# ronghanghu/vit_10b_fsdp_example

Measured on NVIDIA H100. Metric: vit10b images/sec (device-timed, max over ranks), higher is better.
Workload: dtype bf16

## Files before the change

### vit_10b_fsdp_example_b200/csrc/bindings.cpp

```cpp
#include <ATen/cuda/CUDAContext.h>
#include <c10/cuda/CUDAGuard.h>
#include <torch/extension.h>

#include <cmath>
#include <optional>
#include <vector>

#include "attention_sm90.h"
#include "comm.h"
#include "elementwise.h"
#include "gemm_sm90.h"
#include "layer_scale.h"
#include "patch_drop.h"
#include "prefix_tokens.h"

namespace {

using torch::Tensor;
using OptT = std::optional<Tensor>;

inline const __nv_bfloat16* bf16_ptr(const Tensor& t) {
    TORCH_CHECK(t.is_cuda(), "expected a CUDA tensor");
    TORCH_CHECK(t.scalar_type() == at::kBFloat16, "expected a bf16 tensor");
    return reinterpret_cast<const __nv_bfloat16*>(t.data_ptr());
}
inline __nv_bfloat16* bf16_mut(Tensor& t) { return const_cast<__nv_bfloat16*>(bf16_ptr(t)); }
inline float* f32_ptr(const Tensor& t) {
    TORCH_CHECK(t.is_cuda() && t.scalar_type() == at::kFloat, "expected a CUDA fp32 tensor");
    return reinterpret_cast<float*>(t.data_ptr());
}
inline cudaStream_t cur_stream() { return at::cuda::getCurrentCUDAStream().stream(); }

void gemm(Tensor a, int64_t lda, int64_t major_a, Tensor b, int64_t ldb, int64_t major_b, Tensor d, int64_t ldd,
          int64_t M, int64_t N, int64_t K, OptT bias, OptT residual, int64_t ld_res, int64_t res_row_mod, OptT aux_in,
          int64_t ld_aux, OptT aux_out, int64_t ld_aux_out, OptT colsum, int64_t colsum_bi_stride, int64_t act,
          std::vector<int64_t> batch, int64_t block_n, int64_t cluster, int64_t max_ctas, std::vector<int64_t> ag,
          OptT row_scale, int64_t rows_per_scale) {
    c10::cuda::CUDAGuard guard(a.device());
    b200::GemmOperand A, B, D, X;
    A.ptr = bf16_ptr(a), A.ld = lda;
    B.ptr = bf16_ptr(b), B.ld = ldb;
    D.ptr = bf16_ptr(d), D.ld = ldd;
    if (!batch.empty()) {
        TORCH_CHECK(batch.size() == 8, "batch spec must have 8 entries");
        A.nb_inner = B.nb_inner = D.nb_inner = batch[0];
        A.nb_outer = B.nb_outer = D.nb_outer = batch[1];
        A.stride_b_inner = batch[2], A.stride_b_outer = batch[3];
        B.stride_b_inner = batch[4], B.stride_b_outer = batch[5];
        D.stride_b_inner = batch[6], D.stride_b_outer = batch[7];
    }
    b200::GemmEpilogue e;
    if (bias.has_value()) e.bias = bf16_ptr(*bias);
    if (residual.has_value()) e.residual = bf16_ptr(*residual), e.ld_res = ld_res, e.res_row_mod = (int)res_row_mod;
    if (aux_in.has_value()) e.aux_in = bf16_ptr(*aux_in), e.ld_aux = ld_aux;
    if (colsum.has_value()) e.colsum = f32_ptr(*colsum), e.colsum_bi_stride = colsum_bi_stride;
    e.act = static_cast<int>(act);
    if (row_scale.has_value()) {
        TORCH_CHECK(row_scale->is_contiguous() && row_scale->numel() * rows_per_scale >= M,
                    "gemm: row_scale must be contiguous with one entry per rows_per_scale rows");
        e.row_scale = f32_ptr(*row_scale), e.rows_per_scale = (int)rows_per_scale;
    }
    if (aux_out.has_value()) {
        X = D;
        X.ptr = bf16_ptr(*aux_out), X.ld = ld_aux_out;
        e.has_aux_out = 1;
    }
    b200::GemmAgFuse fuse;
    if (!ag.empty()) {
        TORCH_CHECK(ag.size() >= 6 && (int64_t)ag.size() == 6 + ag[0] && ag[0] <= 16, "bad AG-fusion spec");
        fuse.world = (int)ag[0], fuse.rank = (int)ag[1], fuse.rows_per_slab = (int)ag[2], fuse.slab_bytes = ag[3];
        fuse.dst = reinterpret_cast<void*>(ag[4]);
        fuse.flags = reinterpret_cast<uint32_t*>(ag[5]);
        for (int64_t r = 0; r < ag[0]; ++r) fuse.peer_src[r] = static_cast<uint64_t>(ag[6 + r]);
    }
    b200::gemm_bf16(A, (int)major_a, B, (int)major_b, D, aux_out.has_value() ? &X : nullptr, (int)M, (int)N, (int)K, e,
                    (int)block_n, (int)cluster, (int)max_ctas, cur_stream(), ag.empty() ? nullptr : &fuse);
}

void layernorm_fwd(Tensor x, Tensor gamma, Tensor beta, Tensor y, Tensor mean, Tensor rstd, double eps) {
    c10::cuda::CUDAGuard guard(x.device());
    const int D = (int)x.size(-1);
    const int rows = (int)(x.numel() / D);
    b200::layernorm_fwd(bf16_ptr(x), bf16_ptr(gamma), bf16_ptr(beta), bf16_mut(y), f32_ptr(mean), f32_ptr(rstd), rows,
                        D, (float)eps, cur_stream());
}

void layernorm_bwd(Tensor dy, Tensor x, Tensor gamma, Tensor mean, Tensor rstd, OptT dres, Tensor dx, Tensor dgamma,
                   Tensor dbeta, OptT dxsum) {
    c10::cuda::CUDAGuard guard(x.device());
    const int D = (int)x.size(-1);
    const int rows = (int)(x.numel() / D);
    b200::layernorm_bwd(bf16_ptr(dy), bf16_ptr(x), bf16_ptr(gamma), f32_ptr(mean), f32_ptr(rstd),
                        dres.has_value() ? bf16_ptr(*dres) : nullptr, bf16_mut(dx), f32_ptr(dgamma), f32_ptr(dbeta),
                        dxsum.has_value() ? f32_ptr(*dxsum) : nullptr, rows, D, cur_stream());
}

void softmax_fwd(Tensor s, int64_t rows, int64_t n, int64_t ld, double scale) {
    c10::cuda::CUDAGuard guard(s.device());
    b200::softmax_fwd(bf16_mut(s), rows, (int)n, ld, (float)scale, cur_stream());
}
void softmax_bwd(Tensor dp, Tensor p, int64_t rows, int64_t n, int64_t ld, double scale) {
    c10::cuda::CUDAGuard guard(p.device());
    b200::softmax_bwd(bf16_mut(dp), bf16_ptr(p), rows, (int)n, ld, (float)scale, cur_stream());
}

bool attention_supported(int64_t N, int64_t hd) { return b200::attention_supported((int)N, (int)hd); }

void attention_fwd(Tensor qkv, Tensor out, OptT lse, OptT probs, int64_t B, int64_t N, int64_t H, int64_t hd,
                   double drop_p, int64_t drop_key) {
// ... 488 lines not shown
```

### vit_10b_fsdp_example_b200/csrc/gemm_sm90.cu

```cuda
#include <cuda.h>
#include <cuda_runtime.h>
#include <cuda_bf16.h>
#include <cstdint>
#include <cstdio>
#include <cstdlib>
#include <cstring>
#include <mutex>
#include <stdexcept>
#include <string>
#include <algorithm>
#include <unordered_map>

#include "gemm_sm90.h"
#include "ptx.cuh"
#include "wgmma.cuh"

namespace b200 {

namespace {

constexpr int kBlockM = 128;
constexpr int kBlockK = 64;
constexpr int kMmaK = 16;
constexpr int kConsumerWgs = 2;
// ... 30 lines not shown
    uint32_t v;
    asm volatile("ld.acquire.gpu.global.u32 %0, [%1];" : "=r"(v) : "l"(ptr) : "memory");
    return v;
}
__device__ __forceinline__ void fence_proxy_async_all() { asm volatile("fence.proxy.async;" ::: "memory"); }

__device__ __forceinline__ float rcp_approx(float x) {
    float r;
    asm("rcp.approx.ftz.f32 %0, %1;" : "=f"(r) : "f"(x));
    return r;
}
__device__ __forceinline__ float erf_as(float z, float& e) {
    const float az = fabsf(z);
    const float t = rcp_approx(fmaf(0.3275911f, az, 1.0f));
    e = __expf(-az * az);
    float poly = fmaf(1.061405429f, t, -1.453152027f);
    poly = fmaf(poly, t, 1.421413741f);
    poly = fmaf(poly, t, -0.284496736f);
    poly = fmaf(poly, t, 0.254829592f);
    const float y = 1.0f - poly * t * e;
    return copysignf(y, z);
}
__device__ __forceinline__ float gelu_erf(float x) {
    float e;
    return 0.5f * x * (1.0f + erf_as(x * 0.70710678118654752f, e));
}
__device__ __forceinline__ float dgelu_erf(float x) {
    float e;
    const float cdf = 0.5f * (1.0f + erf_as(x * 0.70710678118654752f, e));
    return fmaf(x * 0.3989422804014327f, e, cdf);
}
__device__ __forceinline__ float sigmoid_approx(float x) { return rcp_approx(1.0f + __expf(-x)); }

template <int kMajorA, int kMajorB, int BLOCK_N, int kStages, int kClusterM, bool kRowScale, int kGlu>
__device__ __forceinline__ void gemm_bf16_sm90_body(const CUtensorMap& tmap_a, const CUtensorMap& tmap_b,
                                                    const CUtensorMap& tmap_d, const CUtensorMap& tmap_aux,
                                                    const KernelParams& p) {
    constexpr int kABytes = kBlockM * kBlockK * 2;
    constexpr int kBBytes = BLOCK_N * kBlockK * 2;
    constexpr int kStageBytes = kABytes + kBBytes;
    constexpr int kTileN = kGlu == kActSwiglu ? BLOCK_N / 2 : BLOCK_N;
    static_assert(BLOCK_N % 64 == 0 && BLOCK_N <= 256, "epilogue works in 64-column chunks; wgmma N <= 256");
    static_assert(kABytes % 1024 == 0 && kBBytes % 1024 == 0, "swizzle-128B needs 1024 B aligned stages");
    static_assert(kClusterM == 1 || (kClusterM == 2 && BLOCK_N % 128 == 0), "B splits into two 64-row multiples");
    static_assert(kGlu != kActSwiglu || (kMajorA == 0 && kMajorB == 0 && BLOCK_N % 128 == 0 && !kRowScale),
                  "SwiGLU forward: K-major operands, gate / value halves of 64-row multiples");
    static_assert(kGlu != kActDSwiglu || (kMajorA == 0 && kMajorB == 1 && !kRowScale), "dSwiGLU: the fc2 dgrad (NN)");

    extern __shared__ __align__(1024) uint8_t smem[];
    uint8_t* smem_cd = smem;
    uint8_t* smem_a = smem + kCdBufs * kCdBufBytes;
    uint8_t* smem_b = smem_a + kStages * kABytes;
    uint64_t* full_bar = reinterpret_cast<uint64_t*>(smem_b + kStages * kBBytes);
    uint64_t* empty_bar = full_bar + kStages;

    const uint32_t warp_idx = threadIdx.x / 32;
    const uint32_t lane = lane_id();
    const uint32_t wg = warp_idx / 4;
    if (threadIdx.x == 0 && (smem_u32(smem) & 1023u) != 0) __trap();

    if (warp_idx == 0 && elect_one()) {
        prefetch_tmap(&tmap_a);
        prefetch_tmap(&tmap_b);
        prefetch_tmap(&tmap_d);
        if (p.epi.has_aux_out) prefetch_tmap(&tmap_aux);
        for (int i = 0; i < kStages; ++i) {
            mbar_init(&full_bar[i], 1);
            mbar_init(&empty_bar[i], kConsumerWgs * 4 * kClusterM);
        }
        fence_mbar_init();
    }
    if constexpr (kClusterM > 1)
        cluster_sync();
    else
        __syncthreads();

    auto cta_rank = [] { return kClusterM > 1 ? static_cast<int>(cluster_ctarank()) : 0; };
    const int units_per_batch = p.m_units * p.n_tiles;
    const int total_units = units_per_batch * p.batch;
    const int num_kb = (p.K + kBlockK - 1) / kBlockK;
    const int kGroupN = p.group_n;

    auto decode_tile = [&](int t, int& b, int& mt, int& nt) {
        b = t / units_per_batch;
        const int r = t - b * units_per_batch;
        const int per_group = p.m_units * kGroupN;
        const int g = r / per_group;
        const int first_n = g * kGroupN;
        const int gsz = min(kGroupN, p.n_tiles - first_n);
        const int in_g = r - g * per_group;
        mt = (in_g / gsz) * kClusterM + cta_rank();
        nt = first_n + in_g % gsz;
        nt += p.n_rot;
        if (nt >= p.n_tiles) nt -= p.n_tiles;
    };
    const int ag_chunks_per_slab =
        p.ag.world > 1 ? static_cast<int>((p.ag.slab_bytes + kAgChunkBytes - 1) / kAgChunkBytes) : 0;

    if (wg == 0) {
        reg_dealloc<56>();
        if (warp_idx == 0) {
            if (elect_one()) {
                uint32_t stage = 0, phase = 0;
                for (int t = blockIdx.x / kClusterM; t < total_units; t += gridDim.x / kClusterM) {
                    int b, mt, nt;
                    decode_tile(t, b, mt, nt);
                    const int bi = b % p.nb_inner, bo = b / p.nb_inner;
                    const int m_idx = mt * kBlockM;
                    const int n_idx = nt * kTileN;
                    if (p.ag.world > 1) {
                        const int last_row = min(n_idx + BLOCK_N, p.N) - 1;
                        if (last_row >= n_idx) {
                            const int s_lo = min(n_idx / p.ag.rows_per_slab, p.ag.world - 1);
                            const int s_hi = min(last_row / p.ag.rows_per_slab, p.ag.world - 1);
                            for (int sl = s_lo; sl <= s_hi; ++sl) {
                                uint32_t spins = 0;
                                while (ld_acquire_gpu(p.ag.flags + sl) < static_cast<uint32_t>(ag_chunks_per_slab)) {
                                    if (++spins > (1u << 26)) __trap();
                                }
                            }
                            fence_proxy_async_all();
                        }
                    }
                    for (int kb = 0; kb < num_kb; ++kb) {
                        mbar_wait_silent(&empty_bar[stage], phase ^ 1);
                        const int k_idx = kb * kBlockK;
                        uint8_t* sa = smem_a + stage * kABytes;
                        uint8_t* sb = smem_b + stage * kBBytes;
                        mbar_arrive_expect_tx(&full_bar[stage], kStageBytes);
                        if constexpr (kMajorA == 0) {
                            tma_load_4d(&tmap_a, &full_bar[stage], sa, k_idx, m_idx, bi, bo);
                        } else {
#pragma unroll
                            for (int i = 0; i < kBlockM / 64; ++i)
                                tma_load_4d(&tmap_a, &full_bar[stage], sa + i * (64 * kBlockK * 2), m_idx + i * 64,
                                                 k_idx, bi, bo);
                        }
                        if constexpr (kGlu == kActSwiglu) {
                            constexpr int kHalfN = BLOCK_N / 2;
                            if constexpr (kClusterM == 1) {
                                tma_load_4d(&tmap_b, &full_bar[stage], sb, k_idx, n_idx, bi, bo);
                                tma_load_4d(&tmap_b, &full_bar[stage], sb + kHalfN * (kBlockK * 2), k_idx, p.N + n_idx,
                                            bi, bo);
                            } else {
                                const int r = cta_rank();
                                tma_load_4d_multicast(&tmap_b, &full_bar[stage], sb + r * kHalfN * (kBlockK * 2), k_idx,
                                                      n_idx + r * p.N, bi, bo, 0b11);
                            }
                        } else if constexpr (kClusterM == 1) {
                            if constexpr (kMajorB == 0) {
                                tma_load_4d(&tmap_b, &full_bar[stage], sb, k_idx, n_idx, bi, bo);
                            } else {
#pragma unroll
                                for (int i = 0; i < BLOCK_N / 64; ++i)
                                    tma_load_4d(&tmap_b, &full_bar[stage], sb + i * (64 * kBlockK * 2), n_idx + i * 64,
                                                k_idx, bi, bo);
                            }
                        } else {
                            constexpr int kHalfN = BLOCK_N / 2;
                            const int h = cta_rank() * kHalfN;
                            if constexpr (kMajorB == 0) {
                                tma_load_4d_multicast(&tmap_b, &full_bar[stage], sb + h * (kBlockK * 2), k_idx,
                                                      n_idx + h, bi, bo, 0b11);
                            } else {
#pragma unroll
                                for (int i = 0; i < kHalfN / 64; ++i)
                                    tma_load_4d_multicast(&tmap_b, &full_bar[stage],
// ... 32 lines not shown
                    }
                    for (; i < nvec; i += 32) *reinterpret_cast<uint4*>(dst + static_cast<int64_t>(i) * 16) = ld_peer_v4(src + static_cast<int64_t>(i) * 16);
                    __threadfence();
                    __syncwarp();
                    if (lane == 0) red_release_gpu_add(p.ag.flags + sl, 1);
                }
            }
        }
    } else {
        reg_alloc<224>();
        const uint32_t cw = wg - 1;
        const uint32_t etid = threadIdx.x & 127;
        const uint32_t wrow = (warp_idx & 3) * 16 + lane / 4;
        const uint32_t cpair = (lane & 3) * 2;
        const uint32_t bar_id = 1 + cw;
        uint8_t* const grp_buf = smem_cd + cw * 2 * kCdBufBytes;
        const GemmEpilogue& e = p.epi;
        const bool ext_is_aux = e.act == kActDGelu;
        constexpr uint32_t kLbo = kBlockK * 128;
        constexpr uint32_t kKStepA = kMajorA == 0 ? (kMmaK * 2) : (kMmaK * 128);
        constexpr uint32_t kKStepB = kMajorB == 0 ? (kMmaK * 2) : (kMmaK * 128);
        constexpr uint32_t kSlabA = 64 * kBlockK * 2;
        uint32_t stage = 0, phase = 0;
        uint32_t flip = 0;
        float d[BLOCK_N / 2];
        auto release = [&](uint32_t s) {
            if constexpr (kClusterM == 1) {
                mbar_arrive(&empty_bar[s]);
            } else {
#pragma unroll
                for (int c = 0; c < kClusterM; ++c) mbar_arrive_cluster(&empty_bar[s], c);
            }
        };

        for (int t = blockIdx.x / kClusterM; t < total_units; t += gridDim.x / kClusterM) {
            int b, mt, nt;
            decode_tile(t, b, mt, nt);
            const int bi = b % p.nb_inner, bo = b / p.nb_inner;
            const int m0 = mt * kBlockM + cw * 64;
            const int n0 = nt * kTileN;

            uint32_t prev_stage = 0;
            for (int kb = 0; kb < num_kb; ++kb) {
                mbar_wait_silent(&full_bar[stage], phase);
                const uint32_t a_addr = smem_u32(smem_a + stage * kABytes) + cw * kSlabA;
                const uint32_t b_addr = smem_u32(smem_b + stage * kBBytes);
                wgmma_fence();
#pragma unroll
                for (int k = 0; k < kBlockK / kMmaK; ++k) {
                    const uint64_t da = make_wgmma_desc(a_addr + k * kKStepA, kLbo, 1024, 1);
                    const uint64_t db = make_wgmma_desc(b_addr + k * kKStepB, kLbo, 1024, 1);
                    WgmmaSS<BLOCK_N, kMajorA, kMajorB>::mma(d, da, db, (kb > 0 || k > 0) ? 1u : 0u);
                }
                wgmma_commit();
                if (kb > 0) {
                    wgmma_wait<1>();
                    if (lane == 0) release(prev_stage);
                }
                prev_stage = stage;
                stage = (stage + 1 == kStages) ? 0 : stage + 1;
                phase ^= (stage == 0);
            }
            wgmma_wait<0>();
            if (lane == 0) release(prev_stage);

            const int row0 = m0 + static_cast<int>(wrow), row1 = row0 + 8;
            const bool row0_ok = row0 < p.M, row1_ok = row1 < p.M;
            if constexpr (kGlu == kActSwiglu) {
                constexpr int kHalfChunks = BLOCK_N / 128;
                auto gate_value = [&](int c, int j, float (&a)[4], float (&v)[4]) {
#pragma unroll
                    for (int q = 0; q < 4; ++q) a[q] = d[(c * 8 + j) * 4 + q], v[q] = d[((c + kHalfChunks) * 8 + j) * 4 + q];
                };
#pragma unroll
                for (int c = 0; c < kHalfChunks; ++c) {
                    const int ncol0 = n0 + c * 64;
                    if (ncol0 >= p.N) continue;
                    if (e.bias != nullptr) {
#pragma unroll
                        for (int j = 0; j < 8; ++j) {
                            const int col = ncol0 + j * 8 + static_cast<int>(cpair);
                            if (col < p.N) {
                                const uint32_t bg = __ldg(reinterpret_cast<const uint32_t*>(e.bias + col));
                                const uint32_t bv = __ldg(reinterpret_cast<const uint32_t*>(e.bias + p.N + col));
                                float* dg = d + (c * 8 + j) * 4;
                                float* dv = d + ((c + kHalfChunks) * 8 + j) * 4;
                                dg[0] += bf16_lo(bg), dg[1] += bf16_hi(bg), dg[2] += bf16_lo(bg), dg[3] += bf16_hi(bg);
                                dv[0] += bf16_lo(bv), dv[1] += bf16_hi(bv), dv[2] += bf16_lo(bv), dv[3] += bf16_hi(bv);
                            }
                        }
                    }
                    if (e.has_aux_out) {
                        if (etid == 0) tma_store_wait_read<0>();
                        named_bar_sync(bar_id, kEpiThreads);
#pragma unroll
                        for (int j = 0; j < 8; ++j) {
                            float a[4], v[4];
// ... 193 lines not shown
                            s += __bfloat162float(*reinterpret_cast<const __nv_bfloat16*>(ptr));
                        }
                        if (ncol0 + ccol < p.N)
                            atomicAdd(e.colsum + static_cast<int64_t>(bi) * e.colsum_bi_stride + ncol0 + ccol, s);
                    }
                    ++flip;
                }
            }
        }
        if (etid == 0) tma_store_wait<0>();
    }
    if constexpr (kClusterM > 1) {
        __syncwarp();
        cluster_sync();
    }
}

template <int kMajorA, int kMajorB, int BLOCK_N, int kStages, int kClusterM, bool kRowScale>
__global__ void __launch_bounds__(kNumThreads, 1)
    gemm_bf16_sm90_kernel(const __grid_constant__ CUtensorMap tmap_a, const __grid_constant__ CUtensorMap tmap_b,
                          const __grid_constant__ CUtensorMap tmap_d, const __grid_constant__ CUtensorMap tmap_aux,
                          const KernelParams p) {
    gemm_bf16_sm90_body<kMajorA, kMajorB, BLOCK_N, kStages, kClusterM, kRowScale, 0>(tmap_a, tmap_b, tmap_d, tmap_aux, p);
}

template <int kMajorB, int BLOCK_N, int kStages, int kClusterM, int kGlu>
__global__ void __launch_bounds__(kNumThreads, 1)
    gemm_glu_sm90_kernel(const __grid_constant__ CUtensorMap tmap_a, const __grid_constant__ CUtensorMap tmap_b,
                         const __grid_constant__ CUtensorMap tmap_d, const __grid_constant__ CUtensorMap tmap_aux,
                         const KernelParams p) {
    gemm_bf16_sm90_body<0, kMajorB, BLOCK_N, kStages, kClusterM, false, kGlu>(tmap_a, tmap_b, tmap_d, tmap_aux, p);
}

using EncodeFn = CUresult (*)(CUtensorMap*, CUtensorMapDataType, cuuint32_t, void*, const cuuint64_t*,
                              const cuuint64_t*, const cuuint32_t*, const cuuint32_t*, CUtensorMapInterleave,
                              CUtensorMapSwizzle, CUtensorMapL2promotion, CUtensorMapFloatOOBfill);

EncodeFn get_encode_fn() {
    static EncodeFn fn = nullptr;
    static std::once_flag once;
    std::call_once(once, [] {
        void* sym = nullptr;
        cudaDriverEntryPointQueryResult qres;
        cudaError_t err = cudaGetDriverEntryPoint("cuTensorMapEncodeTiled", &sym, cudaEnableDefault, &qres);
        if (err != cudaSuccess || qres != cudaDriverEntryPointSuccess || sym == nullptr)
            throw std::runtime_error("cuTensorMapEncodeTiled not available from the driver");
        fn = reinterpret_cast<EncodeFn>(sym);
    });
    return fn;
}

struct TmapKey {
    uint64_t ptr;
    int64_t d[4];
    int64_t s[3];
    int32_t box[2];
    bool operator==(const TmapKey& o) const { return std::memcmp(this, &o, sizeof(TmapKey)) == 0; }
};
struct TmapKeyHash {
    size_t operator()(const TmapKey& k) const {
        const uint64_t* w = reinterpret_cast<const uint64_t*>(&k);
        size_t h = 1469598103934665603ull;
        for (size_t i = 0; i < sizeof(TmapKey) / 8; ++i) h = (h ^ w[i]) * 1099511628211ull;
        return h;
    }
};
// ... 29 lines not shown
                                   box, estr, CU_TENSOR_MAP_INTERLEAVE_NONE,
                                   swizzle_bytes == 128 ? CU_TENSOR_MAP_SWIZZLE_128B
                                   : swizzle_bytes == 64 ? CU_TENSOR_MAP_SWIZZLE_64B
                                                         : CU_TENSOR_MAP_SWIZZLE_32B,
                                   CU_TENSOR_MAP_L2_PROMOTION_L2_256B, CU_TENSOR_MAP_FLOAT_OOB_FILL_NONE);
    if (res != CUDA_SUCCESS) {
        char msg[256];
        snprintf(msg, sizeof(msg),
                 "cuTensorMapEncodeTiled failed (%d): dims=(%lld,%lld,%lld,%lld) ld=%lld box=(%d,%d)", (int)res,
                 (long long)inner, (long long)outer, (long long)op.nb_inner, (long long)op.nb_outer, (long long)op.ld,
                 box_inner, box_outer);
        throw std::runtime_error(msg);
    }
    std::lock_guard<std::mutex> lock(mu);
    if (cache.size() > 4096) cache.clear();
    cache.emplace(key, tm);
    return tm;
}

int num_sms() {
    static int n = 0;
    if (n == 0) {
        int dev = 0;
        cudaGetDevice(&dev);
        cudaDeviceGetAttribute(&n, cudaDevAttrMultiProcessorCount, dev);
    }
    return n;
}

void check(cudaError_t err, const char* what) {
    if (err != cudaSuccess) throw std::runtime_error(std::string(what) + ": " + cudaGetErrorString(err));
}

template <int kMajorA, int kMajorB, int BLOCK_N, int kStages, int kClusterM, bool kRowScale, int kGlu>
constexpr auto kernel_for() {
    if constexpr (kGlu == 0)
        return gemm_bf16_sm90_kernel<kMajorA, kMajorB, BLOCK_N, kStages, kClusterM, kRowScale>;
    else
        return gemm_glu_sm90_kernel<kMajorB, BLOCK_N, kStages, kClusterM, kGlu>;
}

template <int kMajorA, int kMajorB, int BLOCK_N, int kStages, int kClusterM, bool kRowScale = false, int kGlu = 0>
void launch(const GemmOperand& A, const GemmOperand& B, const GemmOperand& D, const GemmOperand* aux, int M, int N,
            int K, const GemmEpilogue& epi, int max_ctas, cudaStream_t stream, const GemmAgFuse* ag) {
    constexpr int kSmem = kCdBufs * kCdBufBytes + kStages * (kBlockM + BLOCK_N) * kBlockK * 2 + 2 * kStages * 8;
    static_assert(kSmem <= 232448, "shared memory budget exceeded (227 KB per block on sm_90)");
    constexpr int kTileN = kGlu == kActSwiglu ? BLOCK_N / 2 : BLOCK_N;
    auto kern = kernel_for<kMajorA, kMajorB, BLOCK_N, kStages, kClusterM, kRowScale, kGlu>();
    static bool attr_set = false;
    if (!attr_set) {
        check(cudaFuncSetAttribute(kern, cudaFuncAttributeMaxDynamicSharedMemorySize, kSmem), "cudaFuncSetAttribute");
        attr_set = true;
    }
    cudaLaunchConfig_t cfg = {};
    cudaLaunchAttribute cluster_attr;
    cluster_attr.id = cudaLaunchAttributeClusterDimension;
    cluster_attr.val.clusterDim.x = kClusterM, cluster_attr.val.clusterDim.y = 1, cluster_attr.val.clusterDim.z = 1;
    cfg.blockDim = dim3(kNumThreads);
    cfg.dynamicSmemBytes = kSmem;
    cfg.stream = stream;
    cfg.attrs = &cluster_attr;
    cfg.numAttrs = kClusterM > 1 ? 1 : 0;
    static int resident_units = 0;
    if (resident_units == 0) {
        if constexpr (kClusterM == 1) {
            resident_units = num_sms();
        } else {
            cfg.gridDim = dim3(num_sms() / kClusterM * kClusterM);
            check(cudaOccupancyMaxActiveClusters(&resident_units, kern, &cfg), "cudaOccupancyMaxActiveClusters");
            if (resident_units < 1) throw std::runtime_error("gemm: no 2-CTA cluster of this kernel fits an SM pair");
        }
    }
    CUtensorMap ta = kMajorA == 0 ? make_tmap(A, K, M, kBlockK, kBlockM) : make_tmap(A, M, K, 64, kBlockK);
    CUtensorMap tb = kGlu == kActSwiglu ? make_tmap(B, K, 2 * static_cast<int64_t>(N), kBlockK, BLOCK_N / 2)
                     : kMajorB == 0     ? make_tmap(B, K, N, kBlockK, BLOCK_N / kClusterM)
                                        : make_tmap(B, N, K, 64, kBlockK);
    CUtensorMap td = make_tmap(D, N, M, 64, 64);
    CUtensorMap tx = td;
    if (epi.has_aux_out && aux != nullptr) {
        GemmOperand x = *aux;
        if (kGlu == kActSwiglu) x.nb_inner = 2, x.stride_b_inner = N;
        tx = make_tmap(x, N, M, 64, 64);
    }

    KernelParams p;
    p.M = M, p.N = N, p.K = K;
    p.batch = static_cast<int>(D.nb_inner * D.nb_outer);
    p.nb_inner = static_cast<int>(D.nb_inner);
    p.m_tiles = (M + kBlockM - 1) / kBlockM;
    p.m_units = (p.m_tiles + kClusterM - 1) / kClusterM;
    p.n_tiles = (N + kTileN - 1) / kTileN;
    p.epi = epi;
    p.n_rot = 0;
    p.group_n = 2048 / BLOCK_N;
    if (ag != nullptr && ag->world > 1) {
        if (kMajorB != 0 || p.batch != 1) throw std::runtime_error("gemm: AG fusion needs a K-major, un-batched B");
        if (static_cast<int64_t>(ag->rows_per_slab) * K * 2 != ag->slab_bytes || ag->slab_bytes % 16 != 0)
            throw std::runtime_error("gemm: AG fusion needs whole rows per slab");
        p.ag = *ag;
        p.n_rot = static_cast<int>((static_cast<int64_t>(ag->rank) * ag->rows_per_slab) / BLOCK_N) % p.n_tiles;
        cudaMemsetAsync(ag->flags, 0, sizeof(uint32_t) * (ag->world + 1), stream);
    }
    const int64_t total = static_cast<int64_t>(p.m_units) * p.n_tiles * p.batch;
    int units = resident_units;
    if (max_ctas > 0) units = std::min(units, max_ctas / kClusterM);
    units = static_cast<int>(std::max<int64_t>(1, std::min<int64_t>(total, units)));
    cfg.gridDim = dim3(units * kClusterM);
    check(cudaLaunchKernelEx(&cfg, kern, ta, tb, td, tx, p), "gemm launch failed");
    check(cudaGetLastError(), "gemm launch failed");
}

void gemm_glu(const GemmOperand& A, int major_a, const GemmOperand& B, int major_b, const GemmOperand& D,
              const GemmOperand* aux_out, int M, int N, int K, const GemmEpilogue& epi, int block_n, int cluster,
              int max_ctas, cudaStream_t stream, const GemmAgFuse* ag) {
    const bool fwd = epi.act == kActSwiglu;
    if (epi.residual != nullptr) throw std::runtime_error("gemm: SwiGLU epilogues take no residual");
    if (epi.row_scale != nullptr) throw std::runtime_error("gemm: SwiGLU epilogues take no row_scale");
    if (A.nb_inner * A.nb_outer > 1 || B.nb_inner * B.nb_outer > 1 || D.nb_inner * D.nb_outer > 1)
        throw std::runtime_error("gemm: SwiGLU epilogues take no batched operands");
    if (ag != nullptr && ag->world > 1) throw std::runtime_error("gemm: SwiGLU epilogues take no AG fusion");
    if (N % 8 != 0) throw std::runtime_error("gemm: SwiGLU needs N = H' = Hd / 2 to be a multiple of 8 (Hd % 16 == 0)");
    if (fwd) {
        if (major_a != 0 || major_b != 0) throw std::runtime_error("gemm: SwiGLU forward needs K-major A and B");
        if (epi.aux_in != nullptr || epi.colsum != nullptr)
            throw std::runtime_error("gemm: SwiGLU forward takes no aux_in and no column sums");
        if (epi.has_aux_out != (aux_out != nullptr))
            throw std::runtime_error("gemm: SwiGLU forward: has_aux_out and the aux output go together");
    } else {
        if (major_a != 0 || major_b != 1) throw std::runtime_error("gemm: dSwiGLU needs K-major A and MN-major B");
        if (epi.aux_in == nullptr || aux_out == nullptr || !epi.has_aux_out)
            throw std::runtime_error("gemm: dSwiGLU needs aux_in (u) and an aux output (du_val)");
        if (epi.bias != nullptr) throw std::runtime_error("gemm: dSwiGLU takes no bias");
    }
    if (block_n == 0) block_n = 256;
    if (block_n != 128 && block_n != 256) throw std::runtime_error("gemm: SwiGLU block_n must be 128 or 256");
    if (cluster == 0 || max_ctas == 1) cluster = 1;
#define B200_GLU(MB, BN, ST, ACT)                                                                            \
    cluster == 2 ? launch<0, MB, BN, ST, 2, false, ACT>(A, B, D, aux_out, M, N, K, epi, max_ctas, stream, ag) \
                 : launch<0, MB, BN, ST, 1, false, ACT>(A, B, D, aux_out, M, N, K, epi, max_ctas, stream, ag)
    if (fwd)
        block_n == 256 ? B200_GLU(0, 256, 4, kActSwiglu) : B200_GLU(0, 128, 6, kActSwiglu);
    else
        block_n == 256 ? B200_GLU(1, 256, 4, kActDSwiglu) : B200_GLU(1, 128, 6, kActDSwiglu);
#undef B200_GLU
}

}

CUtensorMap make_tensor_map_4d(const GemmOperand& op, int64_t inner, int64_t outer, int box_inner, int box_outer,
                               int swizzle_bytes) {
    return make_tmap(op, inner, outer, box_inner, box_outer, swizzle_bytes);
}

void gemm_bf16(const GemmOperand& A, int major_a, const GemmOperand& B, int major_b, const GemmOperand& D,
               const GemmOperand* aux_out, int M, int N, int K, const GemmEpilogue& epi, int block_n, int cluster,
               int max_ctas, cudaStream_t stream, const GemmAgFuse* ag) {
    if (epi.act == kActSwiglu || epi.act == kActDSwiglu) {
        gemm_glu(A, major_a, B, major_b, D, aux_out, M, N, K, epi, block_n, cluster, max_ctas, stream, ag);
        return;
    }
    if (N % 8 != 0 && (epi.residual || epi.aux_in))
        throw std::runtime_error("gemm: N must be a multiple of 8 when residual/aux_in are used");
    if (epi.act == kActDGelu && (epi.residual != nullptr || epi.aux_in == nullptr))
        throw std::runtime_error("gemm: dGELU epilogue needs aux_in and cannot be combined with a residual");
    if (D.nb_inner * D.nb_outer > 1 && (epi.bias || epi.residual || epi.aux_in))
        throw std::runtime_error("gemm: bias/residual/aux_in are not supported for batched problems");
    if (cluster != 0 && cluster != 1 && cluster != 2) throw std::runtime_error("gemm: cluster must be 0 (auto), 1 or 2");
    if (block_n == 0) block_n = (N > 128) ? 256 : 128;
    if (cluster == 0 || max_ctas == 1) cluster = 1;
    if (epi.row_scale != nullptr) {
        if (epi.rows_per_scale < 1) throw std::runtime_error("gemm: row_scale needs rows_per_scale >= 1");
        if (epi.act != kActNone || epi.has_aux_out || aux_out != nullptr || epi.colsum != nullptr ||
            D.nb_inner * D.nb_outer > 1)
            throw std::runtime_error("gemm: row_scale only with no activation, no aux output, no column sums, unbatched");
        if (major_a != 0 || major_b != 0) throw std::runtime_error("gemm: row_scale needs K-major A and B");
        if (block_n == 256)
            cluster == 2 ? launch<0, 0, 256, 4, 2, true>(A, B, D, aux_out, M, N, K, epi, max_ctas, stream, ag)
                         : launch<0, 0, 256, 4, 1, true>(A, B, D, aux_out, M, N, K, epi, max_ctas, stream, ag);
        else if (block_n == 128)
            cluster == 2 ? launch<0, 0, 128, 6, 2, true>(A, B, D, aux_out, M, N, K, epi, max_ctas, stream, ag)
                         : launch<0, 0, 128, 6, 1, true>(A, B, D, aux_out, M, N, K, epi, max_ctas, stream, ag);
        else
            throw std::runtime_error("gemm: unsupported block_n");
        return;
    }
#define B200_DISPATCH(MA, MB, BN, ST)                                                             \
    if (major_a == MA && major_b == MB && block_n == BN) {                                        \
        if (cluster == 2)                                                                         \
            launch<MA, MB, BN, ST, 2>(A, B, D, aux_out, M, N, K, epi, max_ctas, stream, ag);      \
        else                                                                                      \
            launch<MA, MB, BN, ST, 1>(A, B, D, aux_out, M, N, K, epi, max_ctas, stream, ag);      \
        return;                                                                                   \
    }
    B200_DISPATCH(0, 0, 256, 4)
    B200_DISPATCH(0, 1, 256, 4)
    B200_DISPATCH(1, 1, 256, 4)
    B200_DISPATCH(1, 0, 256, 4)
    B200_DISPATCH(0, 0, 128, 6)
    B200_DISPATCH(0, 1, 128, 6)
    B200_DISPATCH(1, 1, 128, 6)
    B200_DISPATCH(1, 0, 128, 6)
#undef B200_DISPATCH
// ... 5 lines not shown
```

### vit_10b_fsdp_example_b200/csrc/gemm_sm90.h

```cpp
#pragma once
#include <cuda.h>
#include <cuda_runtime.h>
#include <cuda_bf16.h>
#include <cstdint>

namespace b200 {

enum GemmAct : int { kActNone = 0, kActGelu = 1, kActDGelu = 2, kActSwiglu = 3, kActDSwiglu = 4 };


struct GemmOperand {
    const void* ptr = nullptr;
    int64_t ld = 0;
    int64_t nb_inner = 1, stride_b_inner = 0;
    int64_t nb_outer = 1, stride_b_outer = 0;
};

struct GemmEpilogue {
    const __nv_bfloat16* bias = nullptr;
    const __nv_bfloat16* residual = nullptr;
    const __nv_bfloat16* aux_in = nullptr;
    float* colsum = nullptr;
    int64_t ld_res = 0;
    int64_t ld_aux = 0;
    int64_t colsum_bi_stride = 0;
    int res_row_mod = 0;
    int act = kActNone;
    int has_aux_out = 0;
    const float* row_scale = nullptr;
    int rows_per_scale = 0;
};

struct GemmAgFuse {
    int world = 0;
    int rank = 0;
    int rows_per_slab = 0;
    int64_t slab_bytes = 0;
    uint64_t peer_src[16] = {0};
    void* dst = nullptr;
    uint32_t* flags = nullptr;
};

void gemm_bf16(const GemmOperand& A, int major_a, const GemmOperand& B, int major_b, const GemmOperand& D,
               const GemmOperand* aux_out, int M, int N, int K, const GemmEpilogue& epi, int block_n, int cluster,
               int max_ctas, cudaStream_t stream, const GemmAgFuse* ag = nullptr);

CUtensorMap make_tensor_map_4d(const GemmOperand& op, int64_t inner, int64_t outer, int box_inner, int box_outer,
                               int swizzle_bytes);

}
```

### vit_10b_fsdp_example_b200/csrc/ptx.cuh

```cuda
#pragma once
#include <cuda_runtime.h>
#include <cuda_bf16.h>
#include <cstdint>
#include <cstdio>

namespace b200 {

#ifndef B200_SPIN_LIMIT
#define B200_SPIN_LIMIT (1u << 28)
#endif

__device__ __forceinline__ uint32_t smem_u32(const void* p) {
    return static_cast<uint32_t>(__cvta_generic_to_shared(p));
}

__device__ __forceinline__ uint32_t lane_id() {
    uint32_t l;
    asm volatile("mov.u32 %0, %%laneid;" : "=r"(l));
    return l;
}

__device__ __forceinline__ uint32_t cluster_ctarank() {
    uint32_t r;
    asm volatile("mov.u32 %0, %%cluster_ctarank;" : "=r"(r));
// ... 118 lines not shown
}

__device__ __forceinline__ void tma_store_commit() { asm volatile("cp.async.bulk.commit_group;" ::: "memory"); }

template <int N>
__device__ __forceinline__ void tma_store_wait_read() {
    asm volatile("cp.async.bulk.wait_group.read %0;" ::"n"(N) : "memory");
}
template <int N>
__device__ __forceinline__ void tma_store_wait() {
    asm volatile("cp.async.bulk.wait_group %0;" ::"n"(N) : "memory");
}

template <int N>
__device__ __forceinline__ void reg_dealloc() {
    asm volatile("setmaxnreg.dec.sync.aligned.u32 %0;" ::"n"(N));
}
template <int N>
__device__ __forceinline__ void reg_alloc() {
    asm volatile("setmaxnreg.inc.sync.aligned.u32 %0;" ::"n"(N));
}

__device__ __forceinline__ uint32_t pack_bf16x2(float lo, float hi) {
    __nv_bfloat162 v = __floats2bfloat162_rn(lo, hi);
    return *reinterpret_cast<uint32_t*>(&v);
}
__device__ __forceinline__ float bf16_lo(uint32_t v) { return __uint_as_float(v << 16); }
__device__ __forceinline__ float bf16_hi(uint32_t v) { return __uint_as_float(v & 0xFFFF0000u); }

__device__ __forceinline__ void named_bar_sync(uint32_t id, uint32_t nthreads) {
    asm volatile("bar.sync %0, %1;" ::"r"(id), "r"(nthreads) : "memory");
}

__device__ __forceinline__ void st_shared_b32(uint32_t addr, uint32_t a) {
    asm volatile("st.shared.b32 [%0], %1;" ::"r"(addr), "r"(a) : "memory");
}

__device__ __forceinline__ void st_shared_v4(uint32_t addr, uint32_t a, uint32_t b, uint32_t c, uint32_t d) {
    asm volatile("st.shared.v4.b32 [%0], {%1, %2, %3, %4};" ::"r"(addr), "r"(a), "r"(b), "r"(c), "r"(d) : "memory");
}

}
```

### vit_10b_fsdp_example_b200/ops/cuda_ops.py

```python
from __future__ import annotations

from typing import Optional

import torch

from . import native

NAME = "sm100"


class _CountingModule:

    def __init__(self, mod):
        object.__setattr__(self, "_mod", mod)
        object.__setattr__(self, "count", 0)

    def __getattr__(self, name):
        fn = getattr(self._mod, name)
        if not callable(fn):
            return fn

        def wrapped(*a, **k):
            object.__setattr__(self, "count", self.count + 1)
            return fn(*a, **k)

        object.__setattr__(self, name, wrapped)
        return wrapped


_C = _CountingModule(native.load())


def launch_count() -> int:
    return _C.count

ACT_NONE, ACT_GELU, ACT_DGELU, ACT_SWIGLU, ACT_DSWIGLU = 0, 1, 2, 3, 4
import os as _os

FUSE_ACT_MIN_K = int(_os.environ.get("B200_FUSE_ACT_MIN_K", "2048"))
SWIGLU_FWD_MIN_K = 1536
SWIGLU_DGRAD_K = (1536, 2048)

_max_ctas = 0


def set_compute_max_ctas(n: int) -> None:
    global _max_ctas
    _max_ctas = int(n)


_gemm_cluster = 0


def set_gemm_cluster(n: int) -> None:
    global _gemm_cluster
    assert n in (0, 1, 2), n
    _gemm_cluster = int(n)


def _ld(t: torch.Tensor) -> int:
    assert t.dim() == 2 and t.stride(1) == 1, "expected a row-major 2-D (possibly strided) matrix"
    return t.stride(0)


def _pad8(n: int) -> int:
    return (n + 7) // 8 * 8


def _tma_rows(t: torch.Tensor) -> torch.Tensor:
    if t.stride(1) == 1 and t.stride(0) % 8 == 0 and t.data_ptr() % 16 == 0:
        return t
    rows, cols = t.shape
    buf = torch.zeros(rows, _pad8(cols), dtype=t.dtype, device=t.device)
    buf[:, :cols].copy_(t)
    return buf[:, :cols]


def _bias_ok(b: Optional[torch.Tensor]) -> Optional[torch.Tensor]:
    if b is None or b.numel() % 8 == 0:
        return b
    buf = torch.zeros(_pad8(b.numel()), dtype=b.dtype, device=b.device)
    buf[: b.numel()].copy_(b)
    return buf


def gemm_raw(a, lda, major_a, b, ldb, major_b, d, ldd, M, N, K, *, bias=None, residual=None, ld_res=0,
             res_row_mod=0, aux_in=None, ld_aux=0, aux_out=None, ld_aux_out=0, colsum=None, colsum_bi_stride=0,
             act=ACT_NONE, batch=(), block_n=0, cluster=None, max_ctas=None, ag=(), row_scale=None, rows_per_scale=0):
    _C.gemm(a, lda, major_a, b, ldb, major_b, d, ldd, M, N, K, bias, residual, ld_res, res_row_mod, aux_in, ld_aux,
            aux_out, ld_aux_out, colsum, colsum_bi_stride, act, list(batch), block_n,
            _gemm_cluster if cluster is None else cluster, _max_ctas if max_ctas is None else max_ctas, list(ag),
            row_scale, rows_per_scale)


def ln_fwd(x, w, b, eps: float):
    rows = x.shape[0]
    y = torch.empty_like(x)
    mean = torch.empty(rows, dtype=torch.float32, device=x.device)
    rstd = torch.empty(rows, dtype=torch.float32, device=x.device)
    _C.layernorm_fwd(x, w, b, y, mean, rstd, eps)
    return y, mean, rstd


def ln_bwd(dy, x, w, mean, rstd, dres=None, want_dxsum: bool = False):
    D = x.shape[1]
    dx = torch.empty_like(x)
    acc = torch.zeros(3 if want_dxsum else 2, D, dtype=torch.float32, device=x.device)
    _C.layernorm_bwd(dy, x, w, mean, rstd, dres, dx, acc[0], acc[1], acc[2] if want_dxsum else None)
    return dx, acc[0], acc[1], (acc[2] if want_dxsum else None)


def qk_norm_fwd(qkv, H: int, hd: int, wq, bq, wk, bk, eps: float, inplace: bool = False):
    T = qkv.shape[0]
    out = qkv if inplace else torch.empty(T, 3 * H * hd, dtype=qkv.dtype, device=qkv.device)
    mean = torch.empty(T * 2 * H, dtype=torch.float32, device=qkv.device)
    rstd = torch.empty(T * 2 * H, dtype=torch.float32, device=qkv.device)
    _C.qk_norm_fwd(qkv, wq, bq, wk, bk, out, mean, rstd, H, hd, float(eps))
    return out, mean, rstd


def qk_norm_bwd(dqkv, qkv, H: int, hd: int, wq, wk, mean, rstd):
    acc = torch.zeros(4 * hd + 2 * H * hd, dtype=torch.float32, device=qkv.device)
    dwq, dbq, dwk, dbk = acc[:4 * hd].view(4, hd)
    cs = acc[4 * hd:]
    _C.qk_norm_bwd(dqkv, qkv, wq, wk, mean, rstd, dwq, dbq, dwk, dbk, cs, H, hd)
# ... 390 lines not shown
```

Baseline: 154.3.

## Add ping-pong consumer schedule for dGELU GEMMs with 64-row tiles

Adds a ping-pong GEMM variant where the two consumer warpgroups each own alternate 64-row tiles and take turns on the tensor cores through named-barrier ordering, so one warpgroup's epilogue overlaps the other's MMA mainloop. By default it is selected for block_n=256 GEMMs with a dGELU epilogue and then uses a 2-CTA cluster. It adds a schedule parameter plumbed from Python. The trade-off is smaller M tiles, which mean more B-operand traffic per FLOP, plus extra synchronisation between warpgroups.

Result: no change. 153.9, median of 6 (-0.3%).

```diff
diff --git a/vit_10b_fsdp_example_b200/csrc/bindings.cpp b/vit_10b_fsdp_example_b200/csrc/bindings.cpp
--- a/vit_10b_fsdp_example_b200/csrc/bindings.cpp
+++ b/vit_10b_fsdp_example_b200/csrc/bindings.cpp
@@ -35,7 +35,7 @@
           int64_t M, int64_t N, int64_t K, OptT bias, OptT residual, int64_t ld_res, int64_t res_row_mod, OptT aux_in,
           int64_t ld_aux, OptT aux_out, int64_t ld_aux_out, OptT colsum, int64_t colsum_bi_stride, int64_t act,
           std::vector<int64_t> batch, int64_t block_n, int64_t cluster, int64_t max_ctas, std::vector<int64_t> ag,
-          OptT row_scale, int64_t rows_per_scale) {
+          OptT row_scale, int64_t rows_per_scale, int64_t schedule) {
     c10::cuda::CUDAGuard guard(a.device());
     b200::GemmOperand A, B, D, X;
     A.ptr = bf16_ptr(a), A.ld = lda;
@@ -74,7 +74,8 @@
         for (int64_t r = 0; r < ag[0]; ++r) fuse.peer_src[r] = static_cast<uint64_t>(ag[6 + r]);
     }
     b200::gemm_bf16(A, (int)major_a, B, (int)major_b, D, aux_out.has_value() ? &X : nullptr, (int)M, (int)N, (int)K, e,
-                    (int)block_n, (int)cluster, (int)max_ctas, cur_stream(), ag.empty() ? nullptr : &fuse);
+                    (int)block_n, (int)cluster, (int)schedule, (int)max_ctas, cur_stream(),
+                    ag.empty() ? nullptr : &fuse);
 }
 
 void layernorm_fwd(Tensor x, Tensor gamma, Tensor beta, Tensor y, Tensor mean, Tensor rstd, double eps) {
diff --git a/vit_10b_fsdp_example_b200/csrc/gemm_sm90.cu b/vit_10b_fsdp_example_b200/csrc/gemm_sm90.cu
--- a/vit_10b_fsdp_example_b200/csrc/gemm_sm90.cu
+++ b/vit_10b_fsdp_example_b200/csrc/gemm_sm90.cu
@@ -86,11 +86,20 @@
 }
 __device__ __forceinline__ float sigmoid_approx(float x) { return rcp_approx(1.0f + __expf(-x)); }
 
-template <int kMajorA, int kMajorB, int BLOCK_N, int kStages, int kClusterM, bool kRowScale, int kGlu>
+template <int kStages>
+__device__ __forceinline__ void skip_kblocks(uint32_t& stage, uint32_t& phase, int n) {
+    const uint32_t pos = stage + static_cast<uint32_t>(n);
+    stage = pos % kStages;
+    phase ^= (pos / kStages) & 1u;
+}
+
+template <int kMajorA, int kMajorB, int BLOCK_N, int kStages, int kClusterM, bool kRowScale, int kGlu,
+          bool kPingPong = false>
 __device__ __forceinline__ void gemm_bf16_sm90_body(const CUtensorMap& tmap_a, const CUtensorMap& tmap_b,
                                                     const CUtensorMap& tmap_d, const CUtensorMap& tmap_aux,
                                                     const KernelParams& p) {
-    constexpr int kABytes = kBlockM * kBlockK * 2;
+    constexpr int kTileM = kPingPong ? 64 : kBlockM;
+    constexpr int kABytes = kTileM * kBlockK * 2;
     constexpr int kBBytes = BLOCK_N * kBlockK * 2;
     constexpr int kStageBytes = kABytes + kBBytes;
     constexpr int kTileN = kGlu == kActSwiglu ? BLOCK_N / 2 : BLOCK_N;
@@ -100,6 +109,7 @@
     static_assert(kGlu != kActSwiglu || (kMajorA == 0 && kMajorB == 0 && BLOCK_N % 128 == 0 && !kRowScale),
                   "SwiGLU forward: K-major operands, gate / value halves of 64-row multiples");
     static_assert(kGlu != kActDSwiglu || (kMajorA == 0 && kMajorB == 1 && !kRowScale), "dSwiGLU: the fc2 dgrad (NN)");
+    static_assert(!kPingPong || (kGlu == 0 && !kRowScale), "ping-pong: plain and GELU / dGELU epilogues only");
 
     extern __shared__ __align__(1024) uint8_t smem[];
     uint8_t* smem_cd = smem;
@@ -120,7 +130,7 @@
         if (p.epi.has_aux_out) prefetch_tmap(&tmap_aux);
         for (int i = 0; i < kStages; ++i) {
             mbar_init(&full_bar[i], 1);
-            mbar_init(&empty_bar[i], kConsumerWgs * 4 * kClusterM);
+            mbar_init(&empty_bar[i], (kPingPong ? 1 : kConsumerWgs) * 4 * kClusterM);
         }
         fence_mbar_init();
     }
@@ -160,7 +170,7 @@
                     int b, mt, nt;
                     decode_tile(t, b, mt, nt);
                     const int bi = b % p.nb_inner, bo = b / p.nb_inner;
-                    const int m_idx = mt * kBlockM;
+                    const int m_idx = mt * kTileM;
                     const int n_idx = nt * kTileN;
                     if (p.ag.world > 1) {
                         const int last_row = min(n_idx + BLOCK_N, p.N) - 1;
@@ -186,7 +196,7 @@
                             tma_load_4d(&tmap_a, &full_bar[stage], sa, k_idx, m_idx, bi, bo);
                         } else {
 #pragma unroll
-                            for (int i = 0; i < kBlockM / 64; ++i)
+                            for (int i = 0; i < kTileM / 64; ++i)
                                 tma_load_4d(&tmap_a, &full_bar[stage], sa + i * (64 * kBlockK * 2), m_idx + i * 64,
                                                  k_idx, bi, bo);
                         }
@@ -285,18 +295,27 @@
                 for (int c = 0; c < kClusterM; ++c) mbar_arrive_cluster(&empty_bar[s], c);
             }
         };
-
-        for (int t = blockIdx.x / kClusterM; t < total_units; t += gridDim.x / kClusterM) {
+        constexpr uint32_t kOrderBar = 3;
+        if constexpr (kPingPong) {
+            if (cw == 1) skip_kblocks<kStages>(stage, phase, num_kb);
+        }
+
+        for (int t = blockIdx.x / kClusterM + (kPingPong ? cw * (gridDim.x / kClusterM) : 0); t < total_units;
+             t += (kPingPong ? 2 : 1) * (gridDim.x / kClusterM)) {
             int b, mt, nt;
             decode_tile(t, b, mt, nt);
             const int bi = b % p.nb_inner, bo = b / p.nb_inner;
-            const int m0 = mt * kBlockM + cw * 64;
+            const int m0 = mt * kTileM + (kPingPong ? 0 : cw * 64);
             const int n0 = nt * kTileN;
 
+            if constexpr (kPingPong) {
+                if (t > static_cast<int>(blockIdx.x / kClusterM))
+                    named_bar_sync(kOrderBar + cw, 2 * kEpiThreads);
+            }
             uint32_t prev_stage = 0;
             for (int kb = 0; kb < num_kb; ++kb) {
                 mbar_wait_silent(&full_bar[stage], phase);
-                const uint32_t a_addr = smem_u32(smem_a + stage * kABytes) + cw * kSlabA;
+                const uint32_t a_addr = smem_u32(smem_a + stage * kABytes) + (kPingPong ? 0 : cw * kSlabA);
                 const uint32_t b_addr = smem_u32(smem_b + stage * kBBytes);
                 wgmma_fence();
 #pragma unroll
@@ -314,8 +333,13 @@
                 stage = (stage + 1 == kStages) ? 0 : stage + 1;
                 phase ^= (stage == 0);
             }
+            if constexpr (kPingPong) {
+                if (t + static_cast<int>(gridDim.x / kClusterM) < total_units)
+                    named_bar_arrive(kOrderBar + (cw ^ 1), 2 * kEpiThreads);
+            }
             wgmma_wait<0>();
             if (lane == 0) release(prev_stage);
+            if constexpr (kPingPong) skip_kblocks<kStages>(stage, phase, num_kb);
 
             const int row0 = m0 + static_cast<int>(wrow), row1 = row0 + 8;
             const bool row0_ok = row0 < p.M, row1_ok = row1 < p.M;
@@ -575,6 +599,14 @@
     gemm_bf16_sm90_body<0, kMajorB, BLOCK_N, kStages, kClusterM, false, kGlu>(tmap_a, tmap_b, tmap_d, tmap_aux, p);
 }
 
+template <int kMajorA, int kMajorB, int kStages, int kClusterM>
+__global__ void __launch_bounds__(kNumThreads, 1)
+    gemm_bf16_pingpong_sm90_kernel(const __grid_constant__ CUtensorMap tmap_a, const __grid_constant__ CUtensorMap tmap_b,
+                                   const __grid_constant__ CUtensorMap tmap_d, const __grid_constant__ CUtensorMap tmap_aux,
+                                   const KernelParams p) {
+    gemm_bf16_sm90_body<kMajorA, kMajorB, 256, kStages, kClusterM, false, 0, true>(tmap_a, tmap_b, tmap_d, tmap_aux, p);
+}
+
 using EncodeFn = CUresult (*)(CUtensorMap*, CUtensorMapDataType, cuuint32_t, void*, const cuuint64_t*,
                               const cuuint64_t*, const cuuint32_t*, const cuuint32_t*, CUtensorMapInterleave,
                               CUtensorMapSwizzle, CUtensorMapL2promotion, CUtensorMapFloatOOBfill);
@@ -670,21 +702,25 @@
     if (err != cudaSuccess) throw std::runtime_error(std::string(what) + ": " + cudaGetErrorString(err));
 }
 
-template <int kMajorA, int kMajorB, int BLOCK_N, int kStages, int kClusterM, bool kRowScale, int kGlu>
+template <int kMajorA, int kMajorB, int BLOCK_N, int kStages, int kClusterM, bool kRowScale, int kGlu, bool kPingPong>
 constexpr auto kernel_for() {
-    if constexpr (kGlu == 0)
+    if constexpr (kPingPong)
+        return gemm_bf16_pingpong_sm90_kernel<kMajorA, kMajorB, kStages, kClusterM>;
+    else if constexpr (kGlu == 0)
         return gemm_bf16_sm90_kernel<kMajorA, kMajorB, BLOCK_N, kStages, kClusterM, kRowScale>;
     else
         return gemm_glu_sm90_kernel<kMajorB, BLOCK_N, kStages, kClusterM, kGlu>;
 }
 
-template <int kMajorA, int kMajorB, int BLOCK_N, int kStages, int kClusterM, bool kRowScale = false, int kGlu = 0>
+template <int kMajorA, int kMajorB, int BLOCK_N, int kStages, int kClusterM, bool kRowScale = false, int kGlu = 0,
+          bool kPingPong = false>
 void launch(const GemmOperand& A, const GemmOperand& B, const GemmOperand& D, const GemmOperand* aux, int M, int N,
             int K, const GemmEpilogue& epi, int max_ctas, cudaStream_t stream, const GemmAgFuse* ag) {
-    constexpr int kSmem = kCdBufs * kCdBufBytes + kStages * (kBlockM + BLOCK_N) * kBlockK * 2 + 2 * kStages * 8;
+    constexpr int kTileM = kPingPong ? 64 : kBlockM;
+    constexpr int kSmem = kCdBufs * kCdBufBytes + kStages * (kTileM + BLOCK_N) * kBlockK * 2 + 2 * kStages * 8;
     static_assert(kSmem <= 232448, "shared memory budget exceeded (227 KB per block on sm_90)");
     constexpr int kTileN = kGlu == kActSwiglu ? BLOCK_N / 2 : BLOCK_N;
-    auto kern = kernel_for<kMajorA, kMajorB, BLOCK_N, kStages, kClusterM, kRowScale, kGlu>();
+    auto kern = kernel_for<kMajorA, kMajorB, BLOCK_N, kStages, kClusterM, kRowScale, kGlu, kPingPong>();
     static bool attr_set = false;
     if (!attr_set) {
         check(cudaFuncSetAttribute(kern, cudaFuncAttributeMaxDynamicSharedMemorySize, kSmem), "cudaFuncSetAttribute");
@@ -709,7 +745,7 @@
             if (resident_units < 1) throw std::runtime_error("gemm: no 2-CTA cluster of this kernel fits an SM pair");
         }
     }
-    CUtensorMap ta = kMajorA == 0 ? make_tmap(A, K, M, kBlockK, kBlockM) : make_tmap(A, M, K, 64, kBlockK);
+    CUtensorMap ta = kMajorA == 0 ? make_tmap(A, K, M, kBlockK, kTileM) : make_tmap(A, M, K, 64, kBlockK);
     CUtensorMap tb = kGlu == kActSwiglu ? make_tmap(B, K, 2 * static_cast<int64_t>(N), kBlockK, BLOCK_N / 2)
                      : kMajorB == 0     ? make_tmap(B, K, N, kBlockK, BLOCK_N / kClusterM)
                                         : make_tmap(B, N, K, 64, kBlockK);
@@ -725,7 +761,7 @@
     p.M = M, p.N = N, p.K = K;
     p.batch = static_cast<int>(D.nb_inner * D.nb_outer);
     p.nb_inner = static_cast<int>(D.nb_inner);
-    p.m_tiles = (M + kBlockM - 1) / kBlockM;
+    p.m_tiles = (M + kTileM - 1) / kTileM;
     p.m_units = (p.m_tiles + kClusterM - 1) / kClusterM;
     p.n_tiles = (N + kTileN - 1) / kTileN;
     p.epi = epi;
@@ -792,7 +828,8 @@
 
 void gemm_bf16(const GemmOperand& A, int major_a, const GemmOperand& B, int major_b, const GemmOperand& D,
                const GemmOperand* aux_out, int M, int N, int K, const GemmEpilogue& epi, int block_n, int cluster,
-               int max_ctas, cudaStream_t stream, const GemmAgFuse* ag) {
+               int schedule, int max_ctas, cudaStream_t stream, const GemmAgFuse* ag) {
+    if (schedule < 0 || schedule > 2) throw std::runtime_error("gemm: schedule must be 0 (auto), 1 or 2");
     if (epi.act == kActSwiglu || epi.act == kActDSwiglu) {
         gemm_glu(A, major_a, B, major_b, D, aux_out, M, N, K, epi, block_n, cluster, max_ctas, stream, ag);
         return;
@@ -805,7 +842,25 @@
         throw std::runtime_error("gemm: bias/residual/aux_in are not supported for batched problems");
     if (cluster != 0 && cluster != 1 && cluster != 2) throw std::runtime_error("gemm: cluster must be 0 (auto), 1 or 2");
     if (block_n == 0) block_n = (N > 128) ? 256 : 128;
-    if (cluster == 0 || max_ctas == 1) cluster = 1;
+    const bool pingpong = block_n == 256 && epi.row_scale == nullptr &&
+                          (schedule == 2 || (schedule == 0 && epi.act == kActDGelu));
+    if (cluster == 0) cluster = pingpong ? 2 : 1;
+    if (max_ctas == 1) cluster = 1;
+    if (pingpong) {
+#define B200_PINGPONG(MA, MB)                                                                                          \
+    if (major_a == MA && major_b == MB) {                                                                              \
+        if (cluster == 2)                                                                                              \
+            launch<MA, MB, 256, 4, 2, false, 0, true>(A, B, D, aux_out, M, N, K, epi, max_ctas, stream, ag);           \
+        else                                                                                                           \
+            launch<MA, MB, 256, 4, 1, false, 0, true>(A, B, D, aux_out, M, N, K, epi, max_ctas, stream, ag);           \
+        return;                                                                                                        \
+    }
+        B200_PINGPONG(0, 0)
+        B200_PINGPONG(0, 1)
+        B200_PINGPONG(1, 1)
+        B200_PINGPONG(1, 0)
+#undef B200_PINGPONG
+    }
     if (epi.row_scale != nullptr) {
         if (epi.rows_per_scale < 1) throw std::runtime_error("gemm: row_scale needs rows_per_scale >= 1");
         if (epi.act != kActNone || epi.has_aux_out || aux_out != nullptr || epi.colsum != nullptr ||
diff --git a/vit_10b_fsdp_example_b200/csrc/gemm_sm90.h b/vit_10b_fsdp_example_b200/csrc/gemm_sm90.h
--- a/vit_10b_fsdp_example_b200/csrc/gemm_sm90.h
+++ b/vit_10b_fsdp_example_b200/csrc/gemm_sm90.h
@@ -43,7 +43,7 @@
 
 void gemm_bf16(const GemmOperand& A, int major_a, const GemmOperand& B, int major_b, const GemmOperand& D,
                const GemmOperand* aux_out, int M, int N, int K, const GemmEpilogue& epi, int block_n, int cluster,
-               int max_ctas, cudaStream_t stream, const GemmAgFuse* ag = nullptr);
+               int schedule, int max_ctas, cudaStream_t stream, const GemmAgFuse* ag = nullptr);
 
 CUtensorMap make_tensor_map_4d(const GemmOperand& op, int64_t inner, int64_t outer, int box_inner, int box_outer,
                                int swizzle_bytes);
diff --git a/vit_10b_fsdp_example_b200/csrc/ptx.cuh b/vit_10b_fsdp_example_b200/csrc/ptx.cuh
--- a/vit_10b_fsdp_example_b200/csrc/ptx.cuh
+++ b/vit_10b_fsdp_example_b200/csrc/ptx.cuh
@@ -174,6 +174,10 @@
     asm volatile("bar.sync %0, %1;" ::"r"(id), "r"(nthreads) : "memory");
 }
 
+__device__ __forceinline__ void named_bar_arrive(uint32_t id, uint32_t nthreads) {
+    asm volatile("bar.arrive %0, %1;" ::"r"(id), "r"(nthreads) : "memory");
+}
+
 __device__ __forceinline__ void st_shared_b32(uint32_t addr, uint32_t a) {
     asm volatile("st.shared.b32 [%0], %1;" ::"r"(addr), "r"(a) : "memory");
 }
diff --git a/vit_10b_fsdp_example_b200/ops/cuda_ops.py b/vit_10b_fsdp_example_b200/ops/cuda_ops.py
--- a/vit_10b_fsdp_example_b200/ops/cuda_ops.py
+++ b/vit_10b_fsdp_example_b200/ops/cuda_ops.py
@@ -56,6 +56,16 @@
     global _gemm_cluster
     assert n in (0, 1, 2), n
     _gemm_cluster = int(n)
+
+
+_gemm_schedule = 0
+GEMM_PINGPONG = _os.environ.get("B200_GEMM_PINGPONG", "") != "0"
+
+
+def set_gemm_schedule(n: int) -> None:
+    global _gemm_schedule
+    assert n in (0, 1, 2), n
+    _gemm_schedule = int(n)
 
 
 def _ld(t: torch.Tensor) -> int:
@@ -90,7 +100,7 @@
     _C.gemm(a, lda, major_a, b, ldb, major_b, d, ldd, M, N, K, bias, residual, ld_res, res_row_mod, aux_in, ld_aux,
             aux_out, ld_aux_out, colsum, colsum_bi_stride, act, list(batch), block_n,
             _gemm_cluster if cluster is None else cluster, _max_ctas if max_ctas is None else max_ctas, list(ag),
-            row_scale, rows_per_scale)
+            row_scale, rows_per_scale, _gemm_schedule or (0 if GEMM_PINGPONG else 1))
 
 
 def ln_fwd(x, w, b, eps: float):
```
